# dmiruke/find_motion

Hardware: NVIDIA B200
Metric: 1080p frames/sec (whole box) (higher is better)
Workload: dtype u8+f64

## Files before the change

### find_motion_b200/csrc/fm_common.cuh

```cuda
#pragma once

#include <cuda_runtime.h>
#include <stdint.h>

#include <atomic>

#include "../../include/fm_gpu.h"

#define FM_MAX_K 1024
#define FM_TILE_PX 512
#define FM_TILE_WORDS 16
#define FM_TIMING_RING 16384
#define FM_MAX_DEVICES 64

struct StreamState {
    int has_bg;
    int counter;
    int decay;
    int cache_len;
};

struct ResizeTab {
    int *start;
    int *idx;
// ... 41 lines not shown
    float4 *g4w;
    int g4max;
    int2 *uxt, *uyt;
    struct RowsPlan *rows;
    uint8_t *gray;
    uint16_t *hor;
    uint8_t *blur;
    double *bg;
    uint32_t *maskbits;
    uint32_t *maskflat;
    uint32_t *tflat;
    uint32_t *dil;
    uint32_t *fill;
    int *any;
    int *rawrange;
    int *heavy;
    int *ncomp;
    int *ncounted;
    fm_component *comps;
    fm_frame_stats *stats;
    StreamState *state;
    int *errflag;
    int *nvalid;
    int *nvalid_host;
    CclScratch ccl;
    int *spans;
    int last_T;
    bool planes_valid;
    uint8_t *stage_dev[2];
    size_t stage_bytes[2];
    fm_frame_stats *stats_pinned[2];
    int slot_T[2];
    int *err_pinned;
    cudaStream_t own_stream;
    cudaStream_t copy_stream;
    cudaEvent_t ev_copied[2], ev_done[2];
    uint8_t *clip_ring;
    size_t clip_slot_bytes;
    long long *clip_base;
    FmClipCopy *clip_list;
    int *clip_count;
    int clip_sms;
    bool timing;
    cudaEvent_t *evs;
    int ev_pending;
    double t_ms[3];
    int64_t t_calls;
};

extern std::atomic<unsigned long long> g_launches;
int fm_ensure_smem(const void *func, size_t bytes, int device);
void fm_set_error(const char *fmt, ...);

#define FM_CUDA(call)                                                                     \
    do {                                                                                  \
        cudaError_t e_ = (call);                                                          \
        if (e_ != cudaSuccess) {                                                          \
            fm_set_error("%s failed: %s (%s:%d)", #call, cudaGetErrorString(e_), __FILE__, \
                         __LINE__);                                                       \
            return FM_ECUDA;                                                              \
        }                                                                                 \
    } while (0)

#define FM_LAUNCH_CHECK()                                                         \
    do {                                                                          \
        g_launches.fetch_add(1, std::memory_order_relaxed);                       \
        cudaError_t e_ = cudaGetLastError();                                      \
        if (e_ != cudaSuccess) {                                                  \
            fm_set_error("kernel launch failed: %s (%s:%d)", cudaGetErrorString(e_), \
                         __FILE__, __LINE__);                                     \
            return FM_ECUDA;                                                      \
        }                                                                         \
    } while (0)

int fm_launch_frontend(fm_ctx *c, const uint8_t *frames, size_t sstride, size_t fstride, int T,
                       cudaStream_t st);
int fm_launch_temporal(fm_ctx *c, int T, cudaStream_t st);
int fm_launch_fused(fm_ctx *c, const uint8_t *frames, size_t sstride, size_t fstride, int T, cudaStream_t st);
int fm_ccl_configure(fm_ctx *c);
int fm_launch_morph_ccl(fm_ctx *c, int T, cudaStream_t st, fm_frame_stats *stats_out);
int fm_launch_masks(fm_ctx *c, int stream, int n_polys, const int *offs, const int *pts_scaled,
                    int npts, cudaStream_t st);
int fm_launch_bg_export(fm_ctx *c, int stream, double *dst_dev, cudaStream_t st);
int fm_launch_thresh_export(fm_ctx *c, int stream, int t, uint8_t *dst_dev, cudaStream_t st);
int fm_launch_mask_export(fm_ctx *c, int stream, uint8_t *dst_dev, cudaStream_t st);
bool fm_fused_supported(const fm_ctx *c);
size_t fm_wide_plane_bytes(const fm_ctx *c);
int fm_wide_init(fm_ctx *c, const int *taps);
// ... 46 lines not shown
```

### find_motion_b200/csrc/fm_host.cu

```cuda
#include <ctype.h>
#include <math.h>
#include <stdarg.h>
#include <stdio.h>
#include <stdlib.h>
#include <string.h>

#include <algorithm>
#include <map>
#include <mutex>
#include <utility>
#include <vector>

#include <sched.h>
#include <unistd.h>

#include "fm_common.cuh"

std::atomic<unsigned long long> g_launches{0};
static thread_local char g_err[512] = "";

int fm_ensure_smem(const void *func, size_t bytes, int device) {
    static std::mutex mu;
    static std::map<std::pair<const void *, int>, size_t> done;
    std::lock_guard<std::mutex> lk(mu);
// ... 122 lines not shown

extern "C" int fm_ctx_destroy(fm_ctx *c) {
    if (!c) return FM_OK;
    cudaSetDevice(c->cfg.device);
    cudaDeviceSynchronize();
    cudaFree(c->coef); cudaFree(c->wtab); cudaFree(c->uband); cudaFree(c->uband_f); cudaFree(c->gpad);
    cudaFree(c->g4start); cudaFree(c->g4n); cudaFree(c->g4off); cudaFree(c->g4w);
    cudaFree(c->uxt); cudaFree(c->uyt);
    fm_rows_free(c);
    fm_clips_free(c);
    cudaFree(c->xtab.start); cudaFree(c->xtab.idx); cudaFree(c->xtab.wt);
    cudaFree(c->ytab.start); cudaFree(c->ytab.idx); cudaFree(c->ytab.wt);
    cudaFree(c->gray); cudaFree(c->hor); cudaFree(c->blur); cudaFree(c->bg);
    cudaFree(c->maskbits); cudaFree(c->maskflat); cudaFree(c->tflat); cudaFree(c->dil); cudaFree(c->fill);
    cudaFree(c->heavy); cudaFree(c->rawrange); cudaFree(c->ncomp); cudaFree(c->comps); cudaFree(c->stats);
    cudaFree(c->state); cudaFree(c->errflag); cudaFree(c->nvalid);
    free(c->nvalid_host);
    fm_ccl_free(&c->ccl);
    for (int i = 0; i < 2; i++) {
        cudaFree(c->stage_dev[i]);
        if (c->stats_pinned[i]) cudaFreeHost(c->stats_pinned[i]);
        if (c->ev_copied[i]) cudaEventDestroy(c->ev_copied[i]);
        if (c->ev_done[i]) cudaEventDestroy(c->ev_done[i]);
    }
    if (c->err_pinned) cudaFreeHost(c->err_pinned);
    if (c->own_stream) cudaStreamDestroy(c->own_stream);
    if (c->copy_stream) cudaStreamDestroy(c->copy_stream);
    if (c->evs) {
        for (int i = 0; i < 4 * FM_TIMING_RING; i++) cudaEventDestroy(c->evs[i]);
        delete[] c->evs;
    }
    delete c;
    return FM_OK;
}

extern "C" int fm_ctx_create(const fm_config *cfg, fm_ctx **out) {
    if (!cfg || !out) { fm_set_error("null argument"); return FM_EINVAL; }
    *out = nullptr;
    if (cfg->n_streams < 1 || cfg->frame_width < 1 || cfg->frame_height < 1 || cfg->max_frames < 1 ||
        cfg->box_size < 1 || cfg->blur_scale < 1 || cfg->min_box_scale < 1 || cfg->fps < 0) {
        fm_set_error("invalid configuration (streams/geometry/max_frames/box_size/blur_scale/min_box_scale)");
        return FM_EINVAL;
    }
    if (cfg->box_size > cfg->frame_width && !(cfg->flags & FM_FLAG_UPSCALE)) {
        fm_set_error("box_size %d > frame width %d: upscaling resize needs FM_FLAG_UPSCALE", cfg->box_size,
                     cfg->frame_width);
// ... 119 lines not shown
            return fail(FM_ENOMEM);                                                       \
        }                                                                                 \
    } while (0)
    const bool keep = (cfg->flags & FM_FLAG_KEEP_PLANES) != 0;
    const bool need_gray = keep || !c->fused;
    const bool need_blur = keep || !c->fused;
    ALLOC(c->gray, need_gray ? F * c->N : 16);
    ALLOC(c->hor, (c->fused || c->umma) ? 16 : 2 * fm_wide_plane_bytes(c));
    ALLOC(c->blur, need_blur ? F * c->N + 64 : 64);
    const size_t bg_doubles = std::max((size_t)c->S * c->ntiles * FM_TILE_PX,
                                       c->fused ? fm_fused_bg_doubles(c)
                                                : (c->umma ? fm_umma_bg_doubles(c) : (c->wide_fused ? fm_wide_bg_doubles(c) : (size_t)0)));
    ALLOC(c->bg, bg_doubles * sizeof(double));
    ALLOC(c->maskbits, (size_t)c->S * c->h * c->wpr * 4);
    ALLOC(c->maskflat, (size_t)c->S * flatw * 4);
    ALLOC(c->tflat, (F * flatw + FM_TILE_WORDS) * 4);
    ALLOC(c->dil, F * c->h * c->wpr * 4);
    ALLOC(c->fill, F * c->h * c->wpr * 4);
    ALLOC(c->rawrange, F * 6 * sizeof(int));
    c->any = c->rawrange + 2 * F;
    ALLOC(c->ncomp, (F * 2 + 4) * sizeof(int));
    c->ncounted = c->ncomp + F;
    ALLOC(c->heavy, F * sizeof(int));
    ALLOC(c->comps, F * c->maxc * sizeof(fm_component));
    ALLOC(c->stats, F * sizeof(fm_frame_stats));
    ALLOC(c->state, (size_t)c->S * sizeof(StreamState));
    ALLOC(c->errflag, sizeof(int));
    ALLOC(c->nvalid, (size_t)c->S * sizeof(int));
    c->nvalid_host = (int *)malloc((size_t)c->S * sizeof(int));
    if (!c->nvalid_host) { fm_set_error("out of host memory"); return fail(FM_ENOMEM); }
    for (int s = 0; s < c->S; s++) c->nvalid_host[s] = c->Tmax;
    FM_TRY(cudaMemcpy(c->nvalid, c->nvalid_host, (size_t)c->S * sizeof(int), cudaMemcpyHostToDevice));
    FM_TRY(cudaMemset(c->maskbits, 0, (size_t)c->S * c->h * c->wpr * 4));
    FM_TRY(cudaMemset(c->maskflat, 0, (size_t)c->S * flatw * 4));
    FM_TRY(cudaMemset(c->tflat, 0, (F * flatw + FM_TILE_WORDS) * 4));
    FM_TRY(cudaMemset(c->bg, 0, bg_doubles * sizeof(double)));
    FM_TRY(cudaMemset(c->state, 0, (size_t)c->S * sizeof(StreamState)));
    FM_TRY(cudaMemset(c->errflag, 0, sizeof(int)));
    FM_TRY(cudaMemset(c->heavy, 0, F * sizeof(int)));
    int cap = c->w / 4 + 3;
    size_t per_frame = (size_t)c->h * cap * 28 + (size_t)c->h * 4 + 4;
    size_t budget = (size_t)8 << 30;
    int nb = (int)std::min<size_t>(F, std::max<size_t>(1, budget / per_frame));
    if ((rc = fm_ccl_alloc(&c->ccl, nb, c->h, cap))) return fail(rc);
    if ((rc = fm_ccl_configure(c))) return fail(rc);
    if ((cfg->flags & FM_FLAG_DEVICE_CLIPS) && (rc = fm_clips_alloc(c))) return fail(rc);
    FM_TRY(cudaStreamCreateWithFlags(&c->own_stream, cudaStreamNonBlocking));
    FM_TRY(cudaStreamCreateWithFlags(&c->copy_stream, cudaStreamNonBlocking));
    for (int i = 0; i < 2; i++) {
        FM_TRY(cudaEventCreateWithFlags(&c->ev_copied[i], cudaEventDisableTiming));
        FM_TRY(cudaEventCreateWithFlags(&c->ev_done[i], cudaEventDisableTiming));
    }
// ... 4 lines not shown
}

extern "C" int fm_ctx_info(const fm_ctx *c, fm_info *info) {
    if (!c || !info) { fm_set_error("null argument"); return FM_EINVAL; }
    *info = c->info;
    return FM_OK;
}

extern "C" int fm_ctx_reset(fm_ctx *c, int stream) {
    if (!c) { fm_set_error("null context"); return FM_EINVAL; }
    if (stream >= c->S) { fm_set_error("stream %d out of range", stream); return FM_EINVAL; }
    FM_CUDA(cudaSetDevice(c->cfg.device));
    FM_CUDA(cudaDeviceSynchronize());
    if (stream < 0) {
        FM_CUDA(cudaMemset(c->state, 0, (size_t)c->S * sizeof(StreamState)));
        FM_CUDA(cudaMemset(c->errflag, 0, sizeof(int)));
    } else {
        FM_CUDA(cudaMemset(c->state + stream, 0, sizeof(StreamState)));
    }
    return FM_OK;
}

extern "C" int fm_ctx_check(fm_ctx *c) {
    if (!c) { fm_set_error("null context"); return FM_EINVAL; }
    FM_CUDA(cudaSetDevice(c->cfg.device));
    FM_CUDA(cudaDeviceSynchronize());
    int err = 0;
    FM_CUDA(cudaMemcpy(&err, c->errflag, sizeof(int), cudaMemcpyDeviceToHost));
    if (err) {
        FM_CUDA(cudaMemset(c->errflag, 0, sizeof(int)));
        fm_set_error("contour stage: run capacity exceeded (results of the affected frames are not valid)");
        return FM_ERANGE;
    }
// ... 8 lines not shown
    FM_CUDA(cudaDeviceSynchronize());
    int npts = n_polys ? poly_offsets[n_polys] : 0;
    std::vector<int> pts((size_t)npts * 2);
    const double scale = c->info.scale;
    for (int i = 0; i < npts * 2; i++) pts[i] = (int)((double)xy[i] * scale);
    int s0 = stream < 0 ? 0 : stream, s1 = stream < 0 ? c->S : stream + 1;
    for (int s = s0; s < s1; s++) {
        int rc = fm_launch_masks(c, s, n_polys, poly_offsets, pts.data(), npts, 0);
        if (rc) return rc;
    }
    FM_CUDA(cudaDeviceSynchronize());
    return FM_OK;
}

static int timing_drain(fm_ctx *c) {
    for (int i = 0; i < c->ev_pending; i++) {
        cudaEvent_t *ev = c->evs + 4 * i;
        FM_CUDA(cudaEventSynchronize(ev[3]));
        for (int g = 0; g < 3; g++) {
            float ms = 0;
            FM_CUDA(cudaEventElapsedTime(&ms, ev[g], ev[g + 1]));
            c->t_ms[g] += ms;
        }
        c->t_calls++;
    }
    c->ev_pending = 0;
    return FM_OK;
}

static int process(fm_ctx *c, const uint8_t *frames, size_t stream_stride, size_t frame_stride, int n_frames,
// ... 3 lines not shown
        fm_set_error("n_frames %d outside [1, max_frames=%d]", n_frames, c->Tmax);
        return FM_EINVAL;
    }
    FM_CUDA(cudaSetDevice(c->cfg.device));
    cudaStream_t st = (cudaStream_t)cuda_stream;
    int rc;
    {
        bool changed = false;
        for (int s = 0; s < c->S; s++) {
            int v = n_valid ? n_valid[s] : n_frames;
            if (v < 0 || v > n_frames) { fm_set_error("n_valid[%d] = %d outside [0, n_frames=%d]", s, v, n_frames); return FM_EINVAL; }
            if (v != c->nvalid_host[s]) { c->nvalid_host[s] = v; changed = true; }
        }
        if (changed) FM_CUDA(cudaMemcpyAsync(c->nvalid, c->nvalid_host, (size_t)c->S * sizeof(int), cudaMemcpyHostToDevice, st));
    }
    {
        const size_t Fmax = (size_t)c->S * c->Tmax;
        FM_CUDA(cudaMemsetAsync(c->rawrange, 0xFF, Fmax * 6 * sizeof(int), st));
        FM_CUDA(cudaMemsetAsync(c->ncomp, 0, (Fmax * 2 + 4) * sizeof(int), st));
    }
    cudaEvent_t *ev = nullptr;
    if (c->timing) {
        if (c->ev_pending == FM_TIMING_RING && (rc = timing_drain(c))) return rc;
        ev = c->evs + 4 * c->ev_pending++;
        FM_CUDA(cudaEventRecord(ev[0], st));
    }
    if (c->fused) {
        if ((rc = fm_launch_fused(c, frames, stream_stride, frame_stride, n_frames, st))) return rc;
        if (ev) { FM_CUDA(cudaEventRecord(ev[1], st)); FM_CUDA(cudaEventRecord(ev[2], st)); }
    } else {
        if ((rc = fm_launch_frontend(c, frames, stream_stride, frame_stride, n_frames, st))) return rc;
        if (ev) FM_CUDA(cudaEventRecord(ev[1], st));
        if (!c->wide_fused && !c->umma && (rc = fm_launch_temporal(c, n_frames, st))) return rc;
        if (ev) FM_CUDA(cudaEventRecord(ev[2], st));
    }
    if ((rc = fm_launch_morph_ccl(c, n_frames, st, stats_dev))) return rc;
    if (ev) FM_CUDA(cudaEventRecord(ev[3], st));
    if ((c->cfg.flags & FM_FLAG_DEVICE_CLIPS) &&
        (rc = fm_launch_clips(c, frames, stream_stride, frame_stride, n_frames, out, out_stride, st)))
        return rc;
    c->last_T = n_frames;
    c->planes_valid = true;
    return FM_OK;
}

extern "C" int fm_process_ragged(fm_ctx *c, const uint8_t *frames, size_t stream_stride, size_t frame_stride,
                                 int n_frames, const int32_t *n_valid, void *cuda_stream, fm_frame_stats *stats_dev) {
    return process(c, frames, stream_stride, frame_stride, n_frames, n_valid, cuda_stream, stats_dev, nullptr, 0);
}

extern "C" int fm_process_clip(fm_ctx *c, const uint8_t *frames, size_t stream_stride, size_t frame_stride,
// ... 79 lines not shown
    if (c->err_pinned[slot]) {
        c->err_pinned[slot] = 0;
        cudaMemsetAsync(c->errflag, 0, sizeof(int), c->own_stream);
        fm_set_error("contour stage: run capacity exceeded");
        return FM_ERANGE;
    }
    memcpy(stats_host, c->stats_pinned[slot], (size_t)c->S * T * sizeof(fm_frame_stats));
    return FM_OK;
}

extern "C" int fm_submit_reset(fm_ctx *c, int stream) {
    if (!c) { fm_set_error("null context"); return FM_EINVAL; }
    if (stream < 0 || stream >= c->S) { fm_set_error("stream %d out of range", stream); return FM_EINVAL; }
    FM_CUDA(cudaSetDevice(c->cfg.device));
    FM_CUDA(cudaMemsetAsync(c->state + stream, 0, sizeof(StreamState), c->own_stream));
    return FM_OK;
}

extern "C" int fm_process_host(fm_ctx *c, const uint8_t *frames_host, size_t stream_stride, size_t frame_stride,
                               int n_frames, fm_frame_stats *stats_host) {
    if (!c || !frames_host || !stats_host) { fm_set_error("null argument"); return FM_EINVAL; }
    int rc = fm_submit_host(c, 0, frames_host, stream_stride, frame_stride, n_frames, nullptr);
    if (rc) return rc;
    return fm_wait(c, 0, stats_host);
}

static bool parse_cpulist(const char *txt, cpu_set_t *set) {
    CPU_ZERO(set);
    bool any = false;
    const char *p = txt;
// ... 204 lines not shown
    int m = std::min(*n, max_n);
    std::sort(v.begin(), v.begin() + m, [](const fm_component &a, const fm_component &b) {
        if (a.area_x2 != b.area_x2) return a.area_x2 < b.area_x2;
        if (a.x != b.x) return a.x < b.x;
        if (a.y != b.y) return a.y < b.y;
        if (a.w != b.w) return a.w < b.w;
        return a.h < b.h;
    });
    for (int i = 0; i < m; i++) out[i] = v[i];
    return FM_OK;
}

extern "C" int fm_timing_enable(fm_ctx *c, int on) {
    if (!c) return FM_EINVAL;
    FM_CUDA(cudaSetDevice(c->cfg.device));
    if (on && !c->evs) {
        c->evs = new cudaEvent_t[4 * FM_TIMING_RING];
        for (int i = 0; i < 4 * FM_TIMING_RING; i++) FM_CUDA(cudaEventCreate(&c->evs[i]));
    }
    if (!on && c->ev_pending) { int rc = timing_drain(c); if (rc) return rc; }
    c->timing = on != 0;
    return FM_OK;
}
extern "C" int fm_timing_reset(fm_ctx *c) {
    if (!c) return FM_EINVAL;
    if (c->ev_pending) { int rc = timing_drain(c); if (rc) return rc; }
    c->t_ms[0] = c->t_ms[1] = c->t_ms[2] = 0;
    c->t_calls = 0;
    return FM_OK;
}
extern "C" int fm_timing_get(fm_ctx *c, int which, double *ms_total, int64_t *n_calls) {
// ... 8 lines not shown
```

### find_motion_b200/csrc/k_fused.cu

```cuda
#include <cuda.h>

#include "fm_common.cuh"

#define FT_W 128
#ifndef FT_H
#define FT_H 32
#endif
#define FT_PX 16
#define FUSED_WARPS (FT_H / 4)
#define FG_WORDS 36
#define FG_ROWS (FT_H + 4)
#define FH_MB ((FG_ROWS + 15) / 16)
#define FH_ROWS (16 * FH_MB)
#ifndef FUSED_MIN_CTAS
#define FUSED_MIN_CTAS (1024 / (8 * FT_H))
#endif
#define FH_WORDS 68
#define FUSED_THREADS (8 * FT_H)
#define RAW_PITCH 432
#define RAW_BYTES (RAW_PITCH * FG_ROWS)
#define RAW_STAGE ((RAW_BYTES + 127) / 128 * 128)

__device__ __forceinline__ uint32_t smem_u32(const void *p) { return (uint32_t)__cvta_generic_to_shared(p); }
__device__ __forceinline__ void mbar_init(uint64_t *bar, uint32_t count) {
// ... 17 lines not shown
                                            int c3) {
    asm volatile(
        "cp.async.bulk.tensor.4d.shared::cluster.global.tile.mbarrier::complete_tx::bytes [%0], [%1, {%3, %4, %5, %6}], [%2];"
        ::"r"(smem_u32(dst)), "l"(map), "r"(smem_u32(bar)), "r"(c0), "r"(c1), "r"(c2), "r"(c3)
        : "memory");
}

struct FusedParams {
    int T, w, h, wpr;
    const int *nvalid;
    int tilesX, tilesY;
    double *bg;
    const uint32_t *maskbits;
    uint32_t *tbits;
    size_t flatwords;
    const StreamState *state;
    int b0, b1, b2, shift, rnd;
    int threshold;
    double alpha, beta;
    uint8_t *gray_out, *blur_out;
    int *rawrange;
    uint4 bfr[32];
};

static void fused_bfr(FusedParams &p) {
    for (int lane = 0; lane < 32; lane++) {
        const int g = lane >> 2, tq = lane & 3;
        uint32_t v[4];
        for (int nb = 0; nb < 2; nb++)
            for (int r = 0; r < 2; r++) {
                uint32_t x = 0;
// ... 107 lines not shown
                int q = bg8_magic<SAFE>(bg[idx]);
                push_gt(bits, (unsigned)(q - qoff - (int)sv), nthr2);
                bg[idx] = __fma_rn(bg[idx], p.beta, __fma_rn(X, p.alpha, nC));
            } else {
                const double sd = u8_to_f64(sv);
                if (INIT) bg[idx] = sd;
                int q = bg8_magic<SAFE>(bg[idx]);
                push_gt(bits, (unsigned)(q - qoff - (int)sv), nthr2);
                bg[idx] = __fma_rn(bg[idx], p.beta, __dmul_rn(sd, p.alpha));
            }
        }
    }
    return __brev(bits) >> (32 - FT_PX);
}

template <bool KEEP, bool SAFE>
__global__ void __launch_bounds__(FUSED_THREADS, FUSED_MIN_CTAS) k_fused(const __grid_constant__ CUtensorMap tmap, FusedParams p) {
    extern __shared__ __align__(128) unsigned char fsm[];
    unsigned char *raw = fsm;
    uint32_t *sg = reinterpret_cast<uint32_t *>(fsm + 2 * RAW_STAGE);
    uint32_t *sh = sg + FH_ROWS * FG_WORDS;
    uint64_t *bars = reinterpret_cast<uint64_t *>(sh + FH_ROWS * FH_WORDS);
    const int tid = threadIdx.x, lane = tid & 31, warp = tid >> 5;
    const int s = blockIdx.z;
    const int tx = blockIdx.x, ty = blockIdx.y, tile = ty * p.tilesX + tx;
    const int x0 = tx * FT_W, y0 = ty * FT_H;
    const int w = p.w, h = p.h;
    const bool border = (x0 == 0) || (x0 + FT_W >= w) || (y0 == 0) || (y0 + FT_H >= h);
    const bool has_bg = p.state[s].has_bg != 0;
    const int Ts = min(p.T, __ldg(p.nvalid + s));
    if (Ts <= 0) return;

    const int trow = tid >> 3, xg = tid & 7;
    const int px = x0 + 8 * xg, py = y0 + trow;
    double2 *bgt = reinterpret_cast<double2 *>(p.bg) +
                   ((((size_t)s * p.tilesX * p.tilesY + tile) * FUSED_WARPS + warp) * (FT_PX / 2)) * 32 + lane;
    double bg[FT_PX];
    if (has_bg) {
#pragma unroll
        for (int i = 0; i < FT_PX / 2; i++) {
            double2 v = bgt[i * 32];
            bg[2 * i] = v.x;
            bg[2 * i + 1] = v.y;
        }
    }
    uint32_t M = 0;
// ... 106 lines not shown
        else if (p.shift == 8) bits = fused_rows<KEEP, SAFE, false, false, true>(sgw, bg, M, p, bo, vmask);
        else bits = fused_rows<KEEP, SAFE, false, false, false>(sgw, bg, M, p, bo, vmask);
        if (!okA) bits = 0;
        if (!okB) bits &= 0xFFu;
        if (okA) tb[0] = (uint8_t)bits;
        if (okB) tb[8] = (uint8_t)(bits >> 8);
        if (__any_sync(0xffffffffu, bits != 0) && lane == 0) {
            int *rr = p.rawrange + 2 * ((size_t)s * p.T + t);
            atomicMax(rr, min(y0 + 4 * warp + 3, h - 1));
            atomicMax(rr + 1, h - 1 - (y0 + 4 * warp));
        }
        tb += 4 * p.flatwords;
    }
#pragma unroll
    for (int i = 0; i < FT_PX / 2; i++) bgt[i * 32] = make_double2(bg[2 * i], bg[2 * i + 1]);
}

__global__ void k_bg_export_fused(const double *__restrict__ bg, double *__restrict__ dst, int w, int h, int tilesX,
                                  int tilesY, int s) {
    int x = blockIdx.x * blockDim.x + threadIdx.x, y = blockIdx.y;
    if (x >= w) return;
    int tx = x / FT_W, ty = y / FT_H, tile = ty * tilesX + tx;
    int lx = x - tx * FT_W, ly = y - ty * FT_H;
    int tid = ly * 8 + ((lx & 63) >> 3);
    int warp = tid >> 5, lane = tid & 31;
    int idx = 8 * (lx >> 6) + (lx & 7);
    size_t base = ((((size_t)s * tilesX * tilesY + tile) * FUSED_WARPS + warp) * (FT_PX / 2)) * 32;
    dst[(size_t)y * w + x] = bg[(base + (size_t)(idx >> 1) * 32 + lane) * 2 + (idx & 1)];
}

// ... 33 lines not shown
    PFN_encodeTiled enc = fm_tma_encoder();
    if (!enc) { fm_set_error("cuTensorMapEncodeTiled not available"); return FM_ECUDA; }
    CUtensorMap tmap;
    cuuint64_t dims[4] = {(cuuint64_t)c->W * 3 / 4, (cuuint64_t)c->H, (cuuint64_t)T, (cuuint64_t)c->S};
    cuuint64_t strides[3] = {(cuuint64_t)c->W * 3, (cuuint64_t)fstride, (cuuint64_t)(c->S > 1 ? sstride : fstride * T)};
    cuuint32_t box[4] = {RAW_PITCH / 4, FG_ROWS, 1, 1};
    cuuint32_t estr[4] = {1, 1, 1, 1};
    CUresult r = enc(&tmap, CU_TENSOR_MAP_DATA_TYPE_UINT32, 4, (void *)frames, dims, strides, box, estr,
                     CU_TENSOR_MAP_INTERLEAVE_NONE, CU_TENSOR_MAP_SWIZZLE_NONE, CU_TENSOR_MAP_L2_PROMOTION_L2_128B,
                     CU_TENSOR_MAP_FLOAT_OOB_FILL_NONE);
    if (r != CUDA_SUCCESS) { fm_set_error("cuTensorMapEncodeTiled failed (%d)", (int)r); return FM_ECUDA; }
    FusedParams p;
    p.T = T; p.nvalid = c->nvalid;
    p.w = c->w; p.h = c->h; p.wpr = c->wpr;
    p.tilesX = (c->w + FT_W - 1) / FT_W; p.tilesY = (c->h + FT_H - 1) / FT_H;
    p.bg = c->bg; p.maskbits = c->maskbits; p.tbits = c->tflat;
    p.flatwords = (size_t)c->ntiles * FM_TILE_WORDS;
    p.state = c->state;
    int lg;
    if (c->k == 1) { p.b0 = 0; p.b1 = 0; p.b2 = 1; lg = 8; }
    else if (c->k == 3) { p.b0 = 0; p.b1 = 1; p.b2 = 2; lg = 6; }
    else { p.b0 = 1; p.b1 = 4; p.b2 = 6; lg = 4; }
    p.shift = 16 - 2 * lg;
    int r1 = p.shift ? (1 << (p.shift - 1)) : 0;
    p.rnd = r1 | (r1 << 16);
    p.threshold = c->cfg.threshold;
    p.alpha = c->cfg.avg; p.beta = 1.0 - p.alpha;
    p.gray_out = c->gray; p.blur_out = c->blur;
    p.rawrange = c->rawrange;
    const bool keep = (c->cfg.flags & FM_FLAG_KEEP_PLANES) != 0;
    const bool safe = p.alpha >= 0.0 && p.alpha <= 1.0 && p.threshold >= 0;
    fused_bfr(p);
    dim3 grid(p.tilesX, p.tilesY, c->S);
    int rc;
    if ((rc = fm_ensure_smem((const void *)k_fused<true, true>, FUSED_SMEM, c->cfg.device))) return rc;
    if ((rc = fm_ensure_smem((const void *)k_fused<true, false>, FUSED_SMEM, c->cfg.device))) return rc;
    if ((rc = fm_ensure_smem((const void *)k_fused<false, true>, FUSED_SMEM, c->cfg.device))) return rc;
    if ((rc = fm_ensure_smem((const void *)k_fused<false, false>, FUSED_SMEM, c->cfg.device))) return rc;
    if (keep) {
        if (safe) k_fused<true, true><<<grid, FUSED_THREADS, FUSED_SMEM, st>>>(tmap, p);
        else k_fused<true, false><<<grid, FUSED_THREADS, FUSED_SMEM, st>>>(tmap, p);
    } else {
        if (safe) k_fused<false, true><<<grid, FUSED_THREADS, FUSED_SMEM, st>>>(tmap, p);
        else k_fused<false, false><<<grid, FUSED_THREADS, FUSED_SMEM, st>>>(tmap, p);
    }
    FM_LAUNCH_CHECK();
    return FM_OK;
}

int fm_launch_bg_export_fused(fm_ctx *c, int stream, double *dst_dev, cudaStream_t st) {
    dim3 grid((c->w + 127) / 128, c->h);
    k_bg_export_fused<<<grid, 128, 0, st>>>(c->bg, dst_dev, c->w, c->h, (c->w + FT_W - 1) / FT_W,
                                            (c->h + FT_H - 1) / FT_H, stream);
    FM_LAUNCH_CHECK();
    return FM_OK;
}
```

### find_motion_b200/csrc/k_morph_ccl.cu

```cuda
#include "fm_common.cuh"

#define WARPS_PER_BLOCK 8

__device__ __forceinline__ uint32_t ld_word(const uint32_t *row, int j, int wpr) {
    return ((unsigned)j < (unsigned)wpr) ? __ldg(row + j) : 0u;
}

__device__ __forceinline__ uint32_t flat_row_word(const uint32_t *flat, int y, int j, int w, int h, int wpr) {
    if ((unsigned)y >= (unsigned)h || (unsigned)j >= (unsigned)wpr) return 0u;
    long long b0 = (long long)y * w + 32 * j;
    int wi = (int)(b0 >> 5), sh = (int)(b0 & 31);
    uint32_t lo = __ldg(flat + wi);
    uint32_t v = lo;
    if (sh) {
        uint32_t hi = __ldg(flat + wi + 1);
        v = __funnelshift_r(lo, hi, sh);
    }
    int rem = w - 32 * j;
    if (rem < 32) v &= (1u << rem) - 1u;
    return v;
}

template <bool ALIGNED>
__device__ __forceinline__ uint32_t dilate_vor(const uint32_t *__restrict__ flat, int y, int j, int w, int h, int wpr) {
// ... 80 lines not shown
                    if (rem < 32) d &= (1u << rem) - 1u;
                    dplane[(size_t)y * wpr + j] = d;
                    anyw |= d;
                    if (d) { jmax = max(jmax, j); jmin = min(jmin, j); }
                }
            }
            if (__any_sync(0xffffffffu, anyw != 0)) { ymx = max(ymx, y); ymn = min(ymn, y); }
        }
    }
}

template <bool ALIGNED>
__global__ void __launch_bounds__(32 * WARPS_PER_BLOCK) k_dilate(const uint32_t *__restrict__ tflat,
                                                                 uint32_t *__restrict__ dil, int *__restrict__ rowrange,
                                                                 const int *__restrict__ rawrange, int F, int w, int h,
                                                                 int wpr, int flatwords, int T, int t0, int Th) {
    int warp = blockIdx.x * WARPS_PER_BLOCK + (threadIdx.x >> 5);
    int lane = threadIdx.x & 31;
    if (warp >= F * h) return;
    int lf = warp / h, y = warp - lf * h;
    int f = (lf / Th) * T + t0 + lf % Th;
    if (rawrange) {
        int rmax = rawrange[2 * f], rmin = h - 1 - rawrange[2 * f + 1];
        if (rmax < 0 || y < rmin - 3 || y > rmax + 3) return;
    }
    const uint32_t *flat = tflat + (size_t)f * flatwords;
    uint32_t *out = dil + ((size_t)f * h + y) * wpr;
    int jmax = -1, jmin = wpr;
    const uint32_t anyw = dilate_row<ALIGNED>(flat, out, y, w, h, wpr, lane, jmin, jmax);
    if (__any_sync(0xffffffffu, anyw != 0)) {
        jmax = __reduce_max_sync(0xffffffffu, jmax);
// ... 15 lines not shown
    const int *rawrange;
    int *rangeout;
    uint32_t *planeout;
    int flatwords, aligned;
    int cache_words;
    int f0, nf;
    int T, t0, Th;
    int w, h, wpr, cap;
    size_t slots;
    uint16_t *xs, *xe;
    int *rowcnt, *parent, *area2, *bbox;
    int *errflag;
    int *ncomp, *ncounted;
    fm_component *comps;
    int maxc, min_area, max_area;
};

template <bool INVERT>
__device__ __forceinline__ uint32_t plane_word(const uint32_t *row, int j, int w, int wpr) {
    if ((unsigned)j >= (unsigned)wpr) return 0u;
    uint32_t v = __ldcg(row + j);
    if (INVERT) {
        v = ~v;
        int rem = w - 32 * j;
        if (rem < 32) v &= (1u << rem) - 1u;
    }
    return v;
}

template <bool INVERT>
// ... 192 lines not shown
    __syncthreads();
    for (int y = ylo + warp; y <= yhi; y += nw) runs_row<false>(a, a.fill, lf, f, y, lane);
    __syncthreads();
    for (int y = ylo + warp; y <= yhi; y += nw) union_row<true, false>(a, lf, y, ylo, lane);
    __syncthreads();
    for (int y = ylo + warp; y <= yhi; y += nw) stats_row(a, lf, f, y, lane);
    __syncthreads();
    for (int y = ylo + warp; y <= yhi; y += nw) collect_row(a, lf, f, y, lane);
}

struct DecideArgs {
    StreamState *state;
    fm_frame_stats *stats, *stats_out;
    const int *nvalid;
    int *done;
    int S, T, total, cache_frames, min_movement_frames;
};

__device__ __forceinline__ void decide_stream(const DecideArgs &d, const int *ncomp, const int *ncounted, int s) {
    StreamState st = d.state[s];
    const int T = d.T;
    const int Ts = min(T, d.nvalid[s]);
    for (int t = Ts; t < T; t++) {
        fm_frame_stats z = {0, 0, 0, 0, 0, 0, 0, 0};
        d.stats[s * T + t] = z;
        if (d.stats_out) d.stats_out[s * T + t] = z;
    }
    if (Ts <= 0) return;
    for (int tc = 0; tc < Ts; tc += 16) {
        int nco[16], ncd[16];
// ... 26 lines not shown
                st.cache_len = min(st.cache_len + 1, d.cache_frames);
            }
            r.movement = movement ? 1 : 0;
            r.movement_counter = st.counter;
            r.movement_decay = st.decay;
            r.cache_len = st.cache_len;
            d.stats[f] = r;
            if (d.stats_out) d.stats_out[f] = r;
        }
    }
    st.has_bg = 1;
    d.state[s] = st;
}

__global__ void k_decide(DecideArgs d, const int *__restrict__ ncomp, const int *__restrict__ ncounted) {
    int s = blockIdx.x * blockDim.x + threadIdx.x;
    if (s < d.S) decide_stream(d, ncomp, ncounted, s);
}

__global__ void __launch_bounds__(CCL_THREADS, 1) k_ccl_frame(CclArgs a, const int *__restrict__ heavy) {
    const int lf = blockIdx.x, lg = a.f0 + lf, f = (lg / a.Th) * a.T + a.t0 + lg % a.Th;
    if (heavy && !heavy[f]) return;
    int ylo = 0, yhi = a.h - 1;
    bool work = true;
    if (a.rowrange) {
        int ymax = a.rowrange[4 * f], ymin = a.h - 1 - a.rowrange[4 * f + 1];
        if (ymax < 0) work = false;
        ylo = max(ymin - 1, 0);
        yhi = min(ymax + 1, a.h - 1);
    }
    if (work) ccl_frame_global(a, lf, f, ylo, yhi);
}

#define CCL2_THREADS 1024
#define CCL2_WARPS (CCL2_THREADS / 32)
#define CCL2_CAP 4096

struct RunTable {
    int2 *row;
    int *parent;
    uint16_t *xs, *xe;
    uint16_t *rowof;
};

__device__ __forceinline__ int suf_find(int *parent, int x) {
    int p = parent[x];
// ... 308 lines not shown
        jhi = rng[2];
        jlo = a.wpr - 1 - rng[3];
    } else if (a.rowrange) {
        int ymax = a.rowrange[4 * f], ymin = a.h - 1 - a.rowrange[4 * f + 1];
        if (ymax < 0) return false;
        ylo = max(ymin - 1, 0);
        yhi = min(ymax + 1, a.h - 1);
        jhi = a.rowrange[4 * f + 2];
        jlo = a.wpr - 1 - a.rowrange[4 * f + 3];
    }
    return true;
}

__global__ void __launch_bounds__(CCL2_THREADS, 1) k_ccl_frame_smem(CclArgs a, int *__restrict__ heavy) {
    extern __shared__ __align__(16) unsigned char csm[];
    const int lf = blockIdx.x, lg = a.f0 + lf, f = (lg / a.Th) * a.T + a.t0 + lg % a.Th;
    int ylo, yhi, jlo, jhi;
    bool is_heavy = false;
    if (ccl_window(a, f, ylo, yhi, jlo, jhi)) is_heavy = !ccl_frame_lanes(a, csm, f, lf, ylo, yhi, jlo, jhi - jlo + 1);
    if (threadIdx.x == 0) heavy[f] = is_heavy;
}

__global__ void k_bits_to_u8(const uint32_t *__restrict__ plane, uint8_t *__restrict__ dst, int w, int h, int wpr,
                             uint8_t on, const int *__restrict__ rowrange) {
    int x = blockIdx.x * blockDim.x + threadIdx.x, y = blockIdx.y;
    if (x >= w) return;
    bool live = true;
    if (rowrange) live = rowrange[0] >= 0 && y <= rowrange[0] && y >= h - 1 - rowrange[1];
    dst[(size_t)y * w + x] = (live && ((plane[(size_t)y * wpr + (x >> 5)] >> (x & 31)) & 1u)) ? on : 0;
}
// ... 54 lines not shown
    *smem = tables + (room < 128 * 1024 ? room : 128 * 1024);
    *cache_words = (int)((*smem - tables) / 4);
    return true;
}

int fm_ccl_configure(fm_ctx *c) {
    size_t smem = 0;
    int cw = 0;
    if (!ccl_smem_plan(c->h, c->wpr, &smem, &cw)) return FM_OK;
    return fm_ensure_smem((const void *)k_ccl_frame_smem, smem, c->cfg.device);
}

static int ccl_run(const CclScratch &sc, const uint32_t *plane, uint32_t *fill, int *rowrange, int F, int w,
                   int h, int wpr, int *ncomp, int *ncounted, fm_component *comps, int maxc, int min_area,
                   int max_area, int *errflag, int *heavy, int T, int t0, int Th, cudaStream_t st,
                   const uint32_t *raw = nullptr, const int *rawrange = nullptr, int flatwords = 0) {
    for (int f0 = 0; f0 < F; f0 += sc.frames) {
        int nf = F - f0 < sc.frames ? F - f0 : sc.frames;
        CclArgs a;
        a.plane = plane; a.fill = fill; a.rowrange = rowrange;
        a.raw = raw; a.rawrange = rawrange; a.rangeout = rowrange; a.planeout = const_cast<uint32_t *>(plane);
        a.flatwords = flatwords; a.aligned = (w % 32) == 0;
        a.T = T; a.t0 = t0; a.Th = Th;
        a.f0 = f0; a.nf = nf; a.w = w; a.h = h; a.wpr = wpr; a.cap = sc.cap; a.slots = sc.slots;
        a.xs = sc.xs; a.xe = sc.xe; a.rowcnt = sc.rowcnt; a.parent = sc.parent; a.area2 = sc.area2;
        a.bbox = sc.bbox; a.errflag = errflag;
        a.ncomp = ncomp; a.ncounted = ncounted; a.comps = comps; a.maxc = maxc;
        a.min_area = min_area; a.max_area = max_area;
        a.cache_words = 0;
        size_t smem = 0;
        if (heavy && ccl_smem_plan(h, wpr, &smem, &a.cache_words)) {
            int dev = 0;
            FM_CUDA(cudaGetDevice(&dev));
            int rc = fm_ensure_smem((const void *)k_ccl_frame_smem, smem, dev);
            if (rc) return rc;
            k_ccl_frame_smem<<<nf, CCL2_THREADS, smem, st>>>(a, heavy);
            FM_LAUNCH_CHECK();
            if ((size_t)h * (w / 2 + 2) > CCL2_CAP) k_ccl_frame<<<nf, CCL_THREADS, 0, st>>>(a, heavy);
        } else {
            a.raw = nullptr;
            k_ccl_frame<<<nf, CCL_THREADS, 0, st>>>(a, nullptr);
        }
        FM_LAUNCH_CHECK();
    }
    return FM_OK;
}

int fm_launch_morph_ccl(fm_ctx *c, int T, cudaStream_t st, fm_frame_stats *stats_out) {
    const int F = c->S * T;
    size_t smem_plan = 0;
    int cw_plan = 0, rc;
    const bool smem_ok = ccl_smem_plan(c->h, c->wpr, &smem_plan, &cw_plan);
    if (smem_ok && F >= 32) {
        rc = ccl_run(c->ccl, c->dil, c->fill, c->any, F, c->w, c->h, c->wpr, c->ncomp, c->ncounted, c->comps, c->maxc,
                     c->info.min_area, c->info.max_area, c->errflag, c->heavy, T, 0, T, st, c->tflat, c->rawrange,
                     c->ntiles * FM_TILE_WORDS);
    } else {
        int blocks = (F * c->h + WARPS_PER_BLOCK - 1) / WARPS_PER_BLOCK;
        if (c->w % 32 == 0)
            k_dilate<true><<<blocks, 32 * WARPS_PER_BLOCK, 0, st>>>(c->tflat, c->dil, c->any, c->rawrange, F, c->w, c->h,
                                                                   c->wpr, c->ntiles * FM_TILE_WORDS, T, 0, T);
        else
            k_dilate<false><<<blocks, 32 * WARPS_PER_BLOCK, 0, st>>>(c->tflat, c->dil, c->any, c->rawrange, F, c->w, c->h,
                                                                    c->wpr, c->ntiles * FM_TILE_WORDS, T, 0, T);
        FM_LAUNCH_CHECK();
        rc = ccl_run(c->ccl, c->dil, c->fill, c->any, F, c->w, c->h, c->wpr, c->ncomp, c->ncounted, c->comps, c->maxc,
                     c->info.min_area, c->info.max_area, c->errflag, smem_ok ? c->heavy : nullptr, T, 0, T, st);
    }
    if (rc) return rc;
    DecideArgs d;
    d.state = c->state; d.stats = c->stats; d.stats_out = stats_out; d.nvalid = c->nvalid; d.done = nullptr;
    d.S = c->S; d.T = T; d.total = F; d.cache_frames = c->info.cache_frames; d.min_movement_frames = c->info.min_movement_frames;
    k_decide<<<(c->S + 127) / 128, 128, 0, st>>>(d, c->ncomp, c->ncounted);
    FM_LAUNCH_CHECK();
    return FM_OK;
}

namespace {
struct PlaneScratch {
    CclScratch sc{};
    uint8_t *d8 = nullptr;
    uint32_t *pl = nullptr, *fill = nullptr;
    int *cnt = nullptr;
    fm_component *comps = nullptr;
    ~PlaneScratch() {
        cudaFree(d8); cudaFree(pl); cudaFree(fill); cudaFree(cnt); cudaFree(comps);
        fm_ccl_free(&sc);
    }
// ... 35 lines not shown
```

Measured before the change: 336,100.

## Chain fused and CCL kernels with programmatic dependent launch and double-buffered scratch

Launches the fused, CCL and decide kernels with programmatic stream serialization so that each kernel can start before its predecessor finishes, gated by griddepcontrol wait/launch_dependents. The per-call memset of rawrange and ncomp is removed and moved into the tail of the fused kernel. Double-buffered tflat/rawrange slots and a bg_valid ping-pong array replace the read of StreamState, so the next batch's fused kernel can overlap the current CCL. The fallback CCL kernel's grid is capped at a fixed number of CTAs that loop over frames. Timing with events is replaced by globaltimer stamps. Risks include ordering bugs with the overlapping buffers and some added atomics when timing is on.

Measured after the change: 357,500, median of 6. 6.4% higher.

```diff
diff --git a/find_motion_b200/csrc/fm_common.cuh b/find_motion_b200/csrc/fm_common.cuh
--- a/find_motion_b200/csrc/fm_common.cuh
+++ b/find_motion_b200/csrc/fm_common.cuh
@@ -4,6 +4,7 @@
 #include <stdint.h>
 
 #include <atomic>
+#include <utility>
 
 #include "../../include/fm_gpu.h"
 
@@ -79,6 +80,8 @@
     uint32_t *fill;
     int *any;
     int *rawrange;
+    int slot;
+    int *bg_valid;
     int *heavy;
     int *ncomp;
     int *ncounted;
@@ -108,6 +111,8 @@
     int clip_sms;
     bool timing;
     cudaEvent_t *evs;
+    unsigned long long *stamps;
+    unsigned long long *stamp;
     int ev_pending;
     double t_ms[3];
     int64_t t_calls;
@@ -137,6 +142,36 @@
             return FM_ECUDA;                                                      \
         }                                                                         \
     } while (0)
+
+inline uint32_t *fm_tflat(const fm_ctx *c) {
+    return c->tflat + (size_t)c->slot * c->S * c->Tmax * c->ntiles * FM_TILE_WORDS;
+}
+inline int *fm_rawrange(const fm_ctx *c) { return c->rawrange + (size_t)c->slot * 6 * c->S * c->Tmax; }
+
+template <typename... KArgs, typename... Args>
+cudaError_t fm_launch_chained(void (*kernel)(KArgs...), dim3 grid, dim3 block, size_t smem, cudaStream_t st,
+                              Args &&...args) {
+    cudaLaunchAttribute at[1];
+    at[0].id = cudaLaunchAttributeProgrammaticStreamSerialization;
+    at[0].val.programmaticStreamSerializationAllowed = 1;
+    cudaLaunchConfig_t cfg = {};
+    cfg.gridDim = grid; cfg.blockDim = block; cfg.dynamicSmemBytes = smem; cfg.stream = st;
+    cfg.attrs = at; cfg.numAttrs = 1;
+    return cudaLaunchKernelEx(&cfg, kernel, std::forward<Args>(args)...);
+}
+__device__ __forceinline__ unsigned long long fm_globaltimer() {
+    unsigned long long t;
+    asm volatile("mov.u64 %0, %%globaltimer;" : "=l"(t));
+    return t;
+}
+__device__ __forceinline__ void fm_stamp_start(unsigned long long *stamp) {
+    if (stamp && threadIdx.x == 0) atomicMax(stamp, ~fm_globaltimer());
+}
+__device__ __forceinline__ void fm_stamp_end(unsigned long long *stamp) {
+    if (stamp && threadIdx.x == 0) atomicMax(stamp + 1, fm_globaltimer());
+}
+__device__ __forceinline__ void fm_launch_dependents() { asm volatile("griddepcontrol.launch_dependents;" ::: "memory"); }
+__device__ __forceinline__ void fm_wait_predecessor() { asm volatile("griddepcontrol.wait;" ::: "memory"); }
 
 int fm_launch_frontend(fm_ctx *c, const uint8_t *frames, size_t sstride, size_t fstride, int T,
                        cudaStream_t st);
diff --git a/find_motion_b200/csrc/fm_host.cu b/find_motion_b200/csrc/fm_host.cu
--- a/find_motion_b200/csrc/fm_host.cu
+++ b/find_motion_b200/csrc/fm_host.cu
@@ -160,7 +160,7 @@
     cudaFree(c->gray); cudaFree(c->hor); cudaFree(c->blur); cudaFree(c->bg);
     cudaFree(c->maskbits); cudaFree(c->maskflat); cudaFree(c->tflat); cudaFree(c->dil); cudaFree(c->fill);
     cudaFree(c->heavy); cudaFree(c->rawrange); cudaFree(c->ncomp); cudaFree(c->comps); cudaFree(c->stats);
-    cudaFree(c->state); cudaFree(c->errflag); cudaFree(c->nvalid);
+    cudaFree(c->state); cudaFree(c->bg_valid); cudaFree(c->errflag); cudaFree(c->nvalid);
     free(c->nvalid_host);
     fm_ccl_free(&c->ccl);
     for (int i = 0; i < 2; i++) {
@@ -176,6 +176,7 @@
         for (int i = 0; i < 4 * FM_TIMING_RING; i++) cudaEventDestroy(c->evs[i]);
         delete[] c->evs;
     }
+    cudaFree(c->stamps);
     delete c;
     return FM_OK;
 }
@@ -325,10 +326,11 @@
     ALLOC(c->bg, bg_doubles * sizeof(double));
     ALLOC(c->maskbits, (size_t)c->S * c->h * c->wpr * 4);
     ALLOC(c->maskflat, (size_t)c->S * flatw * 4);
-    ALLOC(c->tflat, (F * flatw + FM_TILE_WORDS) * 4);
+    const size_t slots = c->fused ? 2 : 1;
+    ALLOC(c->tflat, (slots * F * flatw + FM_TILE_WORDS) * 4);
     ALLOC(c->dil, F * c->h * c->wpr * 4);
     ALLOC(c->fill, F * c->h * c->wpr * 4);
-    ALLOC(c->rawrange, F * 6 * sizeof(int));
+    ALLOC(c->rawrange, F * (4 + 2 * slots) * sizeof(int));
     c->any = c->rawrange + 2 * F;
     ALLOC(c->ncomp, (F * 2 + 4) * sizeof(int));
     c->ncounted = c->ncomp + F;
@@ -336,6 +338,7 @@
     ALLOC(c->comps, F * c->maxc * sizeof(fm_component));
     ALLOC(c->stats, F * sizeof(fm_frame_stats));
     ALLOC(c->state, (size_t)c->S * sizeof(StreamState));
+    ALLOC(c->bg_valid, 2 * (size_t)c->S * sizeof(int));
     ALLOC(c->errflag, sizeof(int));
     ALLOC(c->nvalid, (size_t)c->S * sizeof(int));
     c->nvalid_host = (int *)malloc((size_t)c->S * sizeof(int));
@@ -344,9 +347,12 @@
     FM_TRY(cudaMemcpy(c->nvalid, c->nvalid_host, (size_t)c->S * sizeof(int), cudaMemcpyHostToDevice));
     FM_TRY(cudaMemset(c->maskbits, 0, (size_t)c->S * c->h * c->wpr * 4));
     FM_TRY(cudaMemset(c->maskflat, 0, (size_t)c->S * flatw * 4));
-    FM_TRY(cudaMemset(c->tflat, 0, (F * flatw + FM_TILE_WORDS) * 4));
+    FM_TRY(cudaMemset(c->tflat, 0, (slots * F * flatw + FM_TILE_WORDS) * 4));
     FM_TRY(cudaMemset(c->bg, 0, bg_doubles * sizeof(double)));
     FM_TRY(cudaMemset(c->state, 0, (size_t)c->S * sizeof(StreamState)));
+    FM_TRY(cudaMemset(c->bg_valid, 0, 2 * (size_t)c->S * sizeof(int)));
+    FM_TRY(cudaMemset(c->rawrange, 0xFF, F * (4 + 2 * slots) * sizeof(int)));
+    FM_TRY(cudaMemset(c->ncomp, 0, (F * 2 + 4) * sizeof(int)));
     FM_TRY(cudaMemset(c->errflag, 0, sizeof(int)));
     FM_TRY(cudaMemset(c->heavy, 0, F * sizeof(int)));
     int cap = c->w / 4 + 3;
@@ -381,9 +387,11 @@
     FM_CUDA(cudaDeviceSynchronize());
     if (stream < 0) {
         FM_CUDA(cudaMemset(c->state, 0, (size_t)c->S * sizeof(StreamState)));
+        FM_CUDA(cudaMemset(c->bg_valid, 0, 2 * (size_t)c->S * sizeof(int)));
         FM_CUDA(cudaMemset(c->errflag, 0, sizeof(int)));
     } else {
         FM_CUDA(cudaMemset(c->state + stream, 0, sizeof(StreamState)));
+        for (int i = 0; i < 2; i++) FM_CUDA(cudaMemset(c->bg_valid + (size_t)i * c->S + stream, 0, sizeof(int)));
     }
     return FM_OK;
 }
@@ -422,6 +430,21 @@
 }
 
 static int timing_drain(fm_ctx *c) {
+    if (c->fused) {
+        if (!c->ev_pending) return FM_OK;
+        std::vector<unsigned long long> st((size_t)4 * c->ev_pending);
+        FM_CUDA(cudaDeviceSynchronize());
+        FM_CUDA(cudaMemcpy(st.data(), c->stamps, st.size() * sizeof(unsigned long long), cudaMemcpyDeviceToHost));
+        FM_CUDA(cudaMemset(c->stamps, 0, st.size() * sizeof(unsigned long long)));
+        for (int i = 0; i < c->ev_pending; i++) {
+            const unsigned long long *q = &st[4 * (size_t)i];
+            c->t_ms[0] += (double)(q[1] - ~q[0]) * 1e-6;
+            c->t_ms[2] += (double)(q[3] - ~q[2]) * 1e-6;
+            c->t_calls++;
+        }
+        c->ev_pending = 0;
+        return FM_OK;
+    }
     for (int i = 0; i < c->ev_pending; i++) {
         cudaEvent_t *ev = c->evs + 4 * i;
         FM_CUDA(cudaEventSynchronize(ev[3]));
@@ -455,27 +478,31 @@
         }
         if (changed) FM_CUDA(cudaMemcpyAsync(c->nvalid, c->nvalid_host, (size_t)c->S * sizeof(int), cudaMemcpyHostToDevice, st));
     }
-    {
+    if (!c->fused) {
         const size_t Fmax = (size_t)c->S * c->Tmax;
         FM_CUDA(cudaMemsetAsync(c->rawrange, 0xFF, Fmax * 6 * sizeof(int), st));
         FM_CUDA(cudaMemsetAsync(c->ncomp, 0, (Fmax * 2 + 4) * sizeof(int), st));
     }
     cudaEvent_t *ev = nullptr;
+    c->stamp = nullptr;
     if (c->timing) {
         if (c->ev_pending == FM_TIMING_RING && (rc = timing_drain(c))) return rc;
-        ev = c->evs + 4 * c->ev_pending++;
-        FM_CUDA(cudaEventRecord(ev[0], st));
+        if (c->fused) c->stamp = c->stamps + 4 * c->ev_pending++;
+        else { ev = c->evs + 4 * c->ev_pending++; FM_CUDA(cudaEventRecord(ev[0], st)); }
     }
     if (c->fused) {
-        if ((rc = fm_launch_fused(c, frames, stream_stride, frame_stride, n_frames, st))) return rc;
-        if (ev) { FM_CUDA(cudaEventRecord(ev[1], st)); FM_CUDA(cudaEventRecord(ev[2], st)); }
+        rc = fm_launch_fused(c, frames, stream_stride, frame_stride, n_frames, st);
+        if (rc) { if (c->stamp) c->ev_pending--; c->stamp = nullptr; return rc; }
     } else {
         if ((rc = fm_launch_frontend(c, frames, stream_stride, frame_stride, n_frames, st))) return rc;
         if (ev) FM_CUDA(cudaEventRecord(ev[1], st));
         if (!c->wide_fused && !c->umma && (rc = fm_launch_temporal(c, n_frames, st))) return rc;
         if (ev) FM_CUDA(cudaEventRecord(ev[2], st));
     }
-    if ((rc = fm_launch_morph_ccl(c, n_frames, st, stats_dev))) return rc;
+    rc = fm_launch_morph_ccl(c, n_frames, st, stats_dev);
+    c->stamp = nullptr;
+    if (rc) return rc;
+    if (c->fused) c->slot ^= 1;
     if (ev) FM_CUDA(cudaEventRecord(ev[3], st));
     if ((c->cfg.flags & FM_FLAG_DEVICE_CLIPS) &&
         (rc = fm_launch_clips(c, frames, stream_stride, frame_stride, n_frames, out, out_stride, st)))
@@ -585,6 +612,8 @@
     if (stream < 0 || stream >= c->S) { fm_set_error("stream %d out of range", stream); return FM_EINVAL; }
     FM_CUDA(cudaSetDevice(c->cfg.device));
     FM_CUDA(cudaMemsetAsync(c->state + stream, 0, sizeof(StreamState), c->own_stream));
+    for (int i = 0; i < 2; i++)
+        FM_CUDA(cudaMemsetAsync(c->bg_valid + (size_t)i * c->S + stream, 0, sizeof(int), c->own_stream));
     return FM_OK;
 }
 
@@ -819,7 +848,11 @@
 extern "C" int fm_timing_enable(fm_ctx *c, int on) {
     if (!c) return FM_EINVAL;
     FM_CUDA(cudaSetDevice(c->cfg.device));
-    if (on && !c->evs) {
+    if (on && c->fused && !c->stamps) {
+        FM_CUDA(cudaMalloc(&c->stamps, (size_t)4 * FM_TIMING_RING * sizeof(unsigned long long)));
+        FM_CUDA(cudaMemset(c->stamps, 0, (size_t)4 * FM_TIMING_RING * sizeof(unsigned long long)));
+    }
+    if (on && !c->fused && !c->evs) {
         c->evs = new cudaEvent_t[4 * FM_TIMING_RING];
         for (int i = 0; i < 4 * FM_TIMING_RING; i++) FM_CUDA(cudaEventCreate(&c->evs[i]));
     }
diff --git a/find_motion_b200/csrc/k_fused.cu b/find_motion_b200/csrc/k_fused.cu
--- a/find_motion_b200/csrc/k_fused.cu
+++ b/find_motion_b200/csrc/k_fused.cu
@@ -55,7 +55,12 @@
     const uint32_t *maskbits;
     uint32_t *tbits;
     size_t flatwords;
-    const StreamState *state;
+    const int *bg_in;
+    int *bg_out;
+    int *clear_ff;
+    int *clear_zero;
+    int n_ff, n_zero;
+    unsigned long long *stamp;
     int b0, b1, b2, shift, rnd;
     int threshold;
     double alpha, beta;
@@ -193,6 +198,17 @@
     return __brev(bits) >> (32 - FT_PX);
 }
 
+__device__ __forceinline__ void fused_exit(const FusedParams &p) {
+    fm_stamp_end(p.stamp);
+    fm_wait_predecessor();
+    const int nthreads = gridDim.x * gridDim.y * gridDim.z * FUSED_THREADS;
+    for (int i = ((blockIdx.z * gridDim.y + blockIdx.y) * gridDim.x + blockIdx.x) * FUSED_THREADS + threadIdx.x;
+         i < p.n_ff + p.n_zero; i += nthreads) {
+        if (i < p.n_ff) p.clear_ff[i] = -1;
+        else p.clear_zero[i - p.n_ff] = 0;
+    }
+}
+
 template <bool KEEP, bool SAFE>
 __global__ void __launch_bounds__(FUSED_THREADS, FUSED_MIN_CTAS) k_fused(const __grid_constant__ CUtensorMap tmap, FusedParams p) {
     extern __shared__ __align__(128) unsigned char fsm[];
@@ -206,9 +222,14 @@
     const int x0 = tx * FT_W, y0 = ty * FT_H;
     const int w = p.w, h = p.h;
     const bool border = (x0 == 0) || (x0 + FT_W >= w) || (y0 == 0) || (y0 + FT_H >= h);
-    const bool has_bg = p.state[s].has_bg != 0;
+    fm_stamp_start(p.stamp);
+    const bool has_bg = p.bg_in[s] != 0;
     const int Ts = min(p.T, __ldg(p.nvalid + s));
-    if (Ts <= 0) return;
+    if (tid == 0 && tx == 0 && ty == 0) p.bg_out[s] = has_bg || Ts > 0;
+    if (Ts <= 0) {
+        fused_exit(p);
+        return;
+    }
 
     const int trow = tid >> 3, xg = tid & 7;
     const int px = x0 + 8 * xg, py = y0 + trow;
@@ -345,6 +366,7 @@
     }
 #pragma unroll
     for (int i = 0; i < FT_PX / 2; i++) bgt[i * 32] = make_double2(bg[2 * i], bg[2 * i + 1]);
+    fused_exit(p);
 }
 
 __global__ void k_bg_export_fused(const double *__restrict__ bg, double *__restrict__ dst, int w, int h, int tilesX,
@@ -408,9 +430,17 @@
     p.T = T; p.nvalid = c->nvalid;
     p.w = c->w; p.h = c->h; p.wpr = c->wpr;
     p.tilesX = (c->w + FT_W - 1) / FT_W; p.tilesY = (c->h + FT_H - 1) / FT_H;
-    p.bg = c->bg; p.maskbits = c->maskbits; p.tbits = c->tflat;
+    p.bg = c->bg; p.maskbits = c->maskbits; p.tbits = fm_tflat(c);
     p.flatwords = (size_t)c->ntiles * FM_TILE_WORDS;
-    p.state = c->state;
+    p.bg_in = c->bg_valid + (size_t)c->slot * c->S;
+    p.bg_out = c->bg_valid + (size_t)(c->slot ^ 1) * c->S;
+    {
+        const int Fmax = c->S * c->Tmax;
+        p.clear_ff = c->rawrange + (c->slot ? 0 : 2 * Fmax);
+        p.n_ff = 6 * Fmax;
+        p.clear_zero = c->ncomp;
+        p.n_zero = 2 * Fmax + 4;
+    }
     int lg;
     if (c->k == 1) { p.b0 = 0; p.b1 = 0; p.b2 = 1; lg = 8; }
     else if (c->k == 3) { p.b0 = 0; p.b1 = 1; p.b2 = 2; lg = 6; }
@@ -421,7 +451,8 @@
     p.threshold = c->cfg.threshold;
     p.alpha = c->cfg.avg; p.beta = 1.0 - p.alpha;
     p.gray_out = c->gray; p.blur_out = c->blur;
-    p.rawrange = c->rawrange;
+    p.rawrange = fm_rawrange(c);
+    p.stamp = c->stamp;
     const bool keep = (c->cfg.flags & FM_FLAG_KEEP_PLANES) != 0;
     const bool safe = p.alpha >= 0.0 && p.alpha <= 1.0 && p.threshold >= 0;
     fused_bfr(p);
@@ -431,13 +462,9 @@
     if ((rc = fm_ensure_smem((const void *)k_fused<true, false>, FUSED_SMEM, c->cfg.device))) return rc;
     if ((rc = fm_ensure_smem((const void *)k_fused<false, true>, FUSED_SMEM, c->cfg.device))) return rc;
     if ((rc = fm_ensure_smem((const void *)k_fused<false, false>, FUSED_SMEM, c->cfg.device))) return rc;
-    if (keep) {
-        if (safe) k_fused<true, true><<<grid, FUSED_THREADS, FUSED_SMEM, st>>>(tmap, p);
-        else k_fused<true, false><<<grid, FUSED_THREADS, FUSED_SMEM, st>>>(tmap, p);
-    } else {
-        if (safe) k_fused<false, true><<<grid, FUSED_THREADS, FUSED_SMEM, st>>>(tmap, p);
-        else k_fused<false, false><<<grid, FUSED_THREADS, FUSED_SMEM, st>>>(tmap, p);
-    }
+    void (*kern)(const CUtensorMap, FusedParams) = keep ? (safe ? k_fused<true, true> : k_fused<true, false>)
+                                                        : (safe ? k_fused<false, true> : k_fused<false, false>);
+    (void)fm_launch_chained(kern, grid, dim3(FUSED_THREADS), FUSED_SMEM, st, tmap, p);
     FM_LAUNCH_CHECK();
     return FM_OK;
 }
diff --git a/find_motion_b200/csrc/k_morph_ccl.cu b/find_motion_b200/csrc/k_morph_ccl.cu
--- a/find_motion_b200/csrc/k_morph_ccl.cu
+++ b/find_motion_b200/csrc/k_morph_ccl.cu
@@ -118,7 +118,9 @@
 __global__ void __launch_bounds__(32 * WARPS_PER_BLOCK) k_dilate(const uint32_t *__restrict__ tflat,
                                                                  uint32_t *__restrict__ dil, int *__restrict__ rowrange,
                                                                  const int *__restrict__ rawrange, int F, int w, int h,
-                                                                 int wpr, int flatwords, int T, int t0, int Th) {
+                                                                 int wpr, int flatwords, int T, int t0, int Th,
+                                                                 unsigned long long *stamp) {
+    fm_stamp_start(stamp);
     int warp = blockIdx.x * WARPS_PER_BLOCK + (threadIdx.x >> 5);
     int lane = threadIdx.x & 31;
     if (warp >= F * h) return;
@@ -164,6 +166,7 @@
     int *ncomp, *ncounted;
     fm_component *comps;
     int maxc, min_area, max_area;
+    unsigned long long *stamp;
 };
 
 template <bool INVERT>
@@ -386,6 +389,7 @@
     fm_frame_stats *stats, *stats_out;
     const int *nvalid;
     int *done;
+    unsigned long long *stamp;
     int S, T, total, cache_frames, min_movement_frames;
 };
 
@@ -442,22 +446,31 @@
 }
 
 __global__ void k_decide(DecideArgs d, const int *__restrict__ ncomp, const int *__restrict__ ncounted) {
+    fm_launch_dependents();
+    fm_wait_predecessor();
     int s = blockIdx.x * blockDim.x + threadIdx.x;
     if (s < d.S) decide_stream(d, ncomp, ncounted, s);
-}
-
+    fm_stamp_end(d.stamp);
+}
+
+#define CCL_FALLBACK_CTAS 16
 __global__ void __launch_bounds__(CCL_THREADS, 1) k_ccl_frame(CclArgs a, const int *__restrict__ heavy) {
-    const int lf = blockIdx.x, lg = a.f0 + lf, f = (lg / a.Th) * a.T + a.t0 + lg % a.Th;
-    if (heavy && !heavy[f]) return;
-    int ylo = 0, yhi = a.h - 1;
-    bool work = true;
-    if (a.rowrange) {
-        int ymax = a.rowrange[4 * f], ymin = a.h - 1 - a.rowrange[4 * f + 1];
-        if (ymax < 0) work = false;
-        ylo = max(ymin - 1, 0);
-        yhi = min(ymax + 1, a.h - 1);
-    }
-    if (work) ccl_frame_global(a, lf, f, ylo, yhi);
+    fm_launch_dependents();
+    fm_stamp_start(a.stamp);
+    fm_wait_predecessor();
+    for (int lf = blockIdx.x; lf < a.nf; lf += gridDim.x) {
+        const int lg = a.f0 + lf, f = (lg / a.Th) * a.T + a.t0 + lg % a.Th;
+        if (heavy && !heavy[f]) continue;
+        int ylo = 0, yhi = a.h - 1;
+        bool work = true;
+        if (a.rowrange) {
+            int ymax = a.rowrange[4 * f], ymin = a.h - 1 - a.rowrange[4 * f + 1];
+            if (ymax < 0) work = false;
+            ylo = max(ymin - 1, 0);
+            yhi = min(ymax + 1, a.h - 1);
+        }
+        if (work) ccl_frame_global(a, lf, f, ylo, yhi);
+    }
 }
 
 #define CCL2_THREADS 1024
@@ -796,6 +809,8 @@
 
 __global__ void __launch_bounds__(CCL2_THREADS, 1) k_ccl_frame_smem(CclArgs a, int *__restrict__ heavy) {
     extern __shared__ __align__(16) unsigned char csm[];
+    fm_launch_dependents();
+    fm_stamp_start(a.stamp);
     const int lf = blockIdx.x, lg = a.f0 + lf, f = (lg / a.Th) * a.T + a.t0 + lg % a.Th;
     int ylo, yhi, jlo, jhi;
     bool is_heavy = false;
@@ -880,7 +895,8 @@
 static int ccl_run(const CclScratch &sc, const uint32_t *plane, uint32_t *fill, int *rowrange, int F, int w,
                    int h, int wpr, int *ncomp, int *ncounted, fm_component *comps, int maxc, int min_area,
                    int max_area, int *errflag, int *heavy, int T, int t0, int Th, cudaStream_t st,
-                   const uint32_t *raw = nullptr, const int *rawrange = nullptr, int flatwords = 0) {
+                   const uint32_t *raw = nullptr, const int *rawrange = nullptr, int flatwords = 0,
+                   unsigned long long *stamp = nullptr) {
     for (int f0 = 0; f0 < F; f0 += sc.frames) {
         int nf = F - f0 < sc.frames ? F - f0 : sc.frames;
         CclArgs a;
@@ -894,6 +910,7 @@
         a.ncomp = ncomp; a.ncounted = ncounted; a.comps = comps; a.maxc = maxc;
         a.min_area = min_area; a.max_area = max_area;
         a.cache_words = 0;
+        a.stamp = stamp;
         size_t smem = 0;
         if (heavy && ccl_smem_plan(h, wpr, &smem, &a.cache_words)) {
             int dev = 0;
@@ -902,10 +919,11 @@
             if (rc) return rc;
             k_ccl_frame_smem<<<nf, CCL2_THREADS, smem, st>>>(a, heavy);
             FM_LAUNCH_CHECK();
-            if ((size_t)h * (w / 2 + 2) > CCL2_CAP) k_ccl_frame<<<nf, CCL_THREADS, 0, st>>>(a, heavy);
+            if ((size_t)h * (w / 2 + 2) > CCL2_CAP)
+                (void)fm_launch_chained(k_ccl_frame, nf < CCL_FALLBACK_CTAS ? nf : CCL_FALLBACK_CTAS, CCL_THREADS, 0, st, a, (const int *)heavy);
         } else {
             a.raw = nullptr;
-            k_ccl_frame<<<nf, CCL_THREADS, 0, st>>>(a, nullptr);
+            (void)fm_launch_chained(k_ccl_frame, nf, CCL_THREADS, 0, st, a, (const int *)nullptr);
         }
         FM_LAUNCH_CHECK();
     }
@@ -917,27 +935,30 @@
     size_t smem_plan = 0;
     int cw_plan = 0, rc;
     const bool smem_ok = ccl_smem_plan(c->h, c->wpr, &smem_plan, &cw_plan);
+    unsigned long long *stamp = c->stamp ? c->stamp + 2 : nullptr;
     if (smem_ok && F >= 32) {
         rc = ccl_run(c->ccl, c->dil, c->fill, c->any, F, c->w, c->h, c->wpr, c->ncomp, c->ncounted, c->comps, c->maxc,
-                     c->info.min_area, c->info.max_area, c->errflag, c->heavy, T, 0, T, st, c->tflat, c->rawrange,
-                     c->ntiles * FM_TILE_WORDS);
+                     c->info.min_area, c->info.max_area, c->errflag, c->heavy, T, 0, T, st, fm_tflat(c), fm_rawrange(c),
+                     c->ntiles * FM_TILE_WORDS, stamp);
     } else {
         int blocks = (F * c->h + WARPS_PER_BLOCK - 1) / WARPS_PER_BLOCK;
         if (c->w % 32 == 0)
-            k_dilate<true><<<blocks, 32 * WARPS_PER_BLOCK, 0, st>>>(c->tflat, c->dil, c->any, c->rawrange, F, c->w, c->h,
-                                                                   c->wpr, c->ntiles * FM_TILE_WORDS, T, 0, T);
+            k_dilate<true><<<blocks, 32 * WARPS_PER_BLOCK, 0, st>>>(fm_tflat(c), c->dil, c->any, fm_rawrange(c), F, c->w, c->h,
+                                                                   c->wpr, c->ntiles * FM_TILE_WORDS, T, 0, T, stamp);
         else
-            k_dilate<false><<<blocks, 32 * WARPS_PER_BLOCK, 0, st>>>(c->tflat, c->dil, c->any, c->rawrange, F, c->w, c->h,
-                                                                    c->wpr, c->ntiles * FM_TILE_WORDS, T, 0, T);
+            k_dilate<false><<<blocks, 32 * WARPS_PER_BLOCK, 0, st>>>(fm_tflat(c), c->dil, c->any, fm_rawrange(c), F, c->w, c->h,
+                                                                    c->wpr, c->ntiles * FM_TILE_WORDS, T, 0, T, stamp);
         FM_LAUNCH_CHECK();
         rc = ccl_run(c->ccl, c->dil, c->fill, c->any, F, c->w, c->h, c->wpr, c->ncomp, c->ncounted, c->comps, c->maxc,
-                     c->info.min_area, c->info.max_area, c->errflag, smem_ok ? c->heavy : nullptr, T, 0, T, st);
+                     c->info.min_area, c->info.max_area, c->errflag, smem_ok ? c->heavy : nullptr, T, 0, T, st, nullptr,
+                     nullptr, 0, stamp);
     }
     if (rc) return rc;
     DecideArgs d;
     d.state = c->state; d.stats = c->stats; d.stats_out = stats_out; d.nvalid = c->nvalid; d.done = nullptr;
+    d.stamp = stamp;
     d.S = c->S; d.T = T; d.total = F; d.cache_frames = c->info.cache_frames; d.min_movement_frames = c->info.min_movement_frames;
-    k_decide<<<(c->S + 127) / 128, 128, 0, st>>>(d, c->ncomp, c->ncounted);
+    (void)fm_launch_chained(k_decide, (c->S + 127) / 128, 128, 0, st, d, (const int *)c->ncomp, (const int *)c->ncounted);
     FM_LAUNCH_CHECK();
     return FM_OK;
 }
```
